# gmlwns2000/sea-attention

Hardware: AMD Instinct MI355X
Metric: tokens/sec + achieved HBM GB/s, OPT-1.3B SEA T=4096 k=64, 1/2/4/8 MI355X (higher is better)
Workload: dtype bf16

## Files before the change

sea-attention_amd/_build.py:

```python
import hashlib
import os
import subprocess
from concurrent.futures import ThreadPoolExecutor

PKG_DIR = os.path.dirname(os.path.abspath(__file__))
CSRC = os.path.join(PKG_DIR, "csrc")
OBJ_DIR = os.path.join(PKG_DIR, "build")
LIB_PATH = os.path.join(PKG_DIR, "libsea_hip.so")
SOURCES = ["sea_topk.hip", "sea_attn.hip", "sea_attn_tile.hip", "sea_attn_keyrange.hip", "sea_attn_bwd.hip", "sea_csr_ops.hip",
           "sea_predictor.hip", "sea_performer.hip", "sea_conv.hip", "sea_mlp.hip", "sea_decode.hip"]
HEADERS = [os.path.join(CSRC, "sea_common.hpp"), os.path.join(CSRC, "sea_attn.hpp"), os.path.join(CSRC, "sea_tail.hpp"),
           os.path.join(CSRC, "sea_convfrag.hpp"),
           os.path.join(os.path.dirname(PKG_DIR), "include", "sea_hip.h")]
COMMON_FLAGS = ["--offload-arch=gfx950", "-O3", "-std=c++17", "-fPIC", "-fno-slp-vectorize", "-Wall", "-Wno-unused-function"]
FILE_FLAGS = {"sea_attn_tile.hip": ["-mllvm", "-amdgpu-mfma-vgpr-form=1"],
              "sea_attn_bwd.hip": ["-mllvm", "-amdgpu-mfma-vgpr-form=1"]}


def _hipcc():
    for c in (os.environ.get("HIPCC"), "/opt/rocm/bin/hipcc", "hipcc"):
        if c and (os.path.isabs(c) and os.path.exists(c) or not os.path.isabs(c)):
            return c
    return "hipcc"

# ... 15 lines not shown
    return bool(_sources()) and all(os.path.exists(os.path.join(CSRC, s)) for s in SOURCES) and all(os.path.exists(h) for h in HEADERS)


def is_stale():
    if not os.path.exists(LIB_PATH):
        return True
    if not sources_present():
        return False
    if not os.path.exists(LIB_PATH + ".sha256"):
        return True
    return open(LIB_PATH + ".sha256").read().strip() != source_hash()


def ensure_built(verbose=False):
    if not is_stale():
        return LIB_PATH
    import fcntl
    with open(LIB_PATH + ".lock", "w") as lk:
        fcntl.flock(lk, fcntl.LOCK_EX)
        try:
            if is_stale():
                build_library(verbose=verbose)
        finally:
            fcntl.flock(lk, fcntl.LOCK_UN)
    return LIB_PATH


def build_library(force=False, extra_flags=(), out=None, verbose=False):
    out = out or LIB_PATH
    if not force and out == LIB_PATH and not is_stale():
        return out
    cc = _hipcc()
    custom = bool(extra_flags) or out != LIB_PATH
    os.makedirs(os.path.join(OBJ_DIR, "custom") if custom else OBJ_DIR, exist_ok=True)

    hdr_bytes = b"".join(open(h, "rb").read() for h in HEADERS)

    def compile_one(src):
        flags = [*COMMON_FLAGS, *FILE_FLAGS.get(src, []), *extra_flags]
        key = hashlib.sha256(open(os.path.join(CSRC, src), "rb").read() + hdr_bytes + repr(flags).encode()).hexdigest()[:16]
        stem = os.path.splitext(src)[0]
        obj = os.path.join(os.path.join(OBJ_DIR, "custom") if custom else OBJ_DIR, f"{stem}.{key}.o")
        if os.path.exists(obj) and not force:
            return obj
        tmp_o = obj + f".tmp.{os.getpid()}"
        cmd = [cc, *flags, "-c", os.path.join(CSRC, src), "-o", tmp_o]
        if verbose:
            print(" ".join(cmd), flush=True)
        subprocess.run(cmd, check=True)
        os.replace(tmp_o, obj)
        for f in os.listdir(OBJ_DIR):
            if f.startswith(stem + ".") and f.endswith(".o") and f != os.path.basename(obj) and not custom:
                try:
                    os.remove(os.path.join(OBJ_DIR, f))
                except OSError:
                    pass
        return obj

    with ThreadPoolExecutor(max_workers=min(8, os.cpu_count() or 1)) as ex:
        objs = list(ex.map(compile_one, _sources()))
    tmp = out + f".tmp.{os.getpid()}"
    cmd = [cc, "--offload-arch=gfx950", "-shared", "-fPIC", *objs, "-o", tmp]
    if verbose:
        print(" ".join(cmd), flush=True)
    subprocess.run(cmd, check=True)
    os.replace(tmp, out)
    if out == LIB_PATH and not extra_flags:
        with open(LIB_PATH + ".sha256", "w") as f:
            f.write(source_hash())
    return out


if __name__ == "__main__":
    print(build_library(force=True, verbose=True))
```

sea-attention_amd/csrc/sea_performer.hip:

```cpp
#include "sea_common.hpp"
#include <cstdlib>

#ifdef SEA_STAMP
__device__ unsigned long long sea_dbg_perf[16];
__device__ unsigned long long sea_dbg_wg[2048];
#define PSTAMP(i) do { if (threadIdx.x == 0) { unsigned long long _t = __builtin_amdgcn_s_memtime(); atomicAdd(&sea_dbg_perf[i], _t - _tprev); _tprev = _t; } } while (0)
#define WSTAMP(i) do { if (threadIdx.x == 0 && (STATE_ONLY || blockIdx.y == 0 || blockIdx.y == gridDim.y - 1)) { unsigned long long _t = __builtin_amdgcn_s_memtime(); _tacc[i] += _t - _tprev; _tprev = _t; } } while (0)
#define WSTAMP_FLUSH() do { if (!STATE_ONLY && threadIdx.x == 0 && (blockIdx.y == 0 || blockIdx.y == gridDim.y - 1)) for (int _i = 0; _i < 4; ++_i) atomicAdd(&sea_dbg_perf[_i + (blockIdx.y ? 0 : 4)], _tacc[_i]); \
    if (STATE_ONLY && threadIdx.x == 0) for (int _i = 0; _i < 4; ++_i) atomicAdd(&sea_dbg_perf[10 + _i], _tacc[_i]); \
    if (threadIdx.x == 0) atomicAdd(&sea_dbg_perf[STATE_ONLY ? 8 : 9], __builtin_amdgcn_s_memtime() - _tstart); \
    if (!STATE_ONLY && threadIdx.x == 0) { const int _w = blockIdx.y * gridDim.x + blockIdx.x; if (_w < 1024) { sea_dbg_wg[2 * _w] = _rstart; sea_dbg_wg[2 * _w + 1] = __builtin_amdgcn_s_memrealtime(); } } } while (0)
#else
#define PSTAMP(i) do {} while (0)
#define WSTAMP(i) do {} while (0)
#define WSTAMP_FLUSH() do {} while (0)
#endif

namespace sea {

using f4 = __attribute__((ext_vector_type(4))) float;
#define SEA_MFMA(a, b, c) __builtin_amdgcn_mfma_f32_16x16x4f32((a), (b), (c), 0, 0, 0)

struct PerfParams {
  const void *q, *k, *v;
// ... 300 lines not shown
    __syncthreads();
    PSTAMP(4);
  }
  if constexpr (STATE_ONLY) {
    float* cw = p.carry + ((int64_t)nh * (p.nseg - 1) + seg) * CARRY;
#pragma unroll
    for (int a = 0; a < JB; ++a)
#pragma unroll
      for (int b = 0; b < NBT; ++b)
#pragma unroll
        for (int r = 0; r < 4; ++r) cw[((a * NBT + b) * 4 + r) * NTH + tid] = S[a][b][r];
    if (tid < NBP) cw[JB * NBT * 4 * NTH + tid] = sKsum[tid];
  } else if (p.state_out && seg == p.nseg - 1) {
    float* cw = p.state_out + (int64_t)nh * CARRY;
#pragma unroll
    for (int a = 0; a < JB; ++a)
#pragma unroll
      for (int b = 0; b < NBT; ++b)
#pragma unroll
        for (int r = 0; r < 4; ++r) cw[((a * NBT + b) * 4 + r) * NTH + tid] = S[a][b][r];
    if (tid < NBP) cw[JB * NBT * 4 * NTH + tid] = sKsum[tid];
  }
}


template <typename T> __device__ inline void split16(float x, unsigned short& hi, unsigned short& lo) {
  hi = S16<T>::bits(x);
  lo = S16<T>::bits(x - S16<T>::val(hi));
}
__device__ inline uint2 pack4(const unsigned short (&v)[4]) {
  return make_uint2((uint32_t)v[0] | ((uint32_t)v[1] << 16), (uint32_t)v[2] | ((uint32_t)v[3] << 16));
}
__device__ inline uint4 cat8(uint2 a, uint2 b) { return make_uint4(a.x, a.y, b.x, b.y); }
__device__ inline uint2 lds_tr(const unsigned short* p) {
  const ps4 v = __builtin_amdgcn_ds_read_tr16_b64_v4i16((ps4 __attribute__((address_space(3)))*)(p));
  return __builtin_bit_cast(uint2, v);
}

template <typename T, int NBT, bool STATE_ONLY, bool SEQ = false, bool PAGED = false>
__global__ __launch_bounds__(512) void performer_bf16_kernel(PerfParams p) {
  constexpr int D = 64, C = 64, NW = 8, NTH = 512, E = 2 * D;
  constexpr int NBP = NBT * 16;
  constexpr int KF = (NBT + 1) / 2;
  constexpr int FP = KF * 32;
  constexpr int RB = C / 16, EB = E / 16;
  static_assert(EB == NW, "one 16-column block of [pos | v] per wave");
  constexpr int LDQ2 = FP + 16;
  constexpr int LDK2 = (FP == 64) ? 96 : FP + 8;
  constexpr int LDA = C + 16;
  constexpr int DSL = RB + NTH / C;
  extern __shared__ __attribute__((aligned(16))) char smem_b[];
  unsigned short* sW = reinterpret_cast<unsigned short*>(smem_b);
  unsigned short* sQ = sW + (D / 8) * NBP * 8;
  unsigned short* sK = sQ + (D / 8) * C * 8;
  unsigned short* sV = sK + (D / 8) * C * 8;
  unsigned short* sQh = sV + C * E;
  unsigned short* sQl = sQh + C * LDQ2;
  unsigned short* sKh = sQl + C * LDQ2;
  unsigned short* sKl = sKh + C * LDK2;
  constexpr int NSET = (FP == 64) ? 2 : 1;
  unsigned short* sAh = sKl + C * LDK2 + (NSET - 1) * (2 * C * LDQ2 + 2 * C * LDK2);
  unsigned short* sAl = sAh + C * LDA;
  float* sKsum = reinterpret_cast<float*>(sAl + C * LDA);
  float* sDenP = sKsum + FP;
  float* sKsP = sDenP + C * DSL;

// ... 99 lines not shown
  auto tril_frag = [&](int ib, int ks) {
    unsigned short o[8];
#pragma unroll
    for (int j = 0; j < 8; ++j) o[j] = (ks * 32 + lg * 8 + j <= ib * 16 + li) ? S16<T>::ONE : (unsigned short)0;
    const unsigned short (&o0)[4] = *reinterpret_cast<const unsigned short (*)[4]>(&o[0]);
    const unsigned short (&o1)[4] = *reinterpret_cast<const unsigned short (*)[4]>(&o[4]);
    return cat8(pack4(o0), pack4(o1));
  };

  uint4 tril[RB][C / 32];
#pragma unroll
  for (int ib = 0; ib < RB; ++ib)
#pragma unroll
    for (int ks = 0; ks < C / 32; ++ks) tril[ib][ks] = tril_frag(ib, ks);

  auto write_state = [&]() {
    float* cw = p.state_out + (int64_t)nh * CARRY;
#pragma unroll
    for (int b = 0; b < NBT; ++b)
#pragma unroll
      for (int r = 0; r < 4; ++r) cw[(b * 4 + r) * NTH + tid] = S[b][r];
    if (tid < FP) cw[NBT * 4 * NTH + tid] = sKsum[tid];
    cw[NBT * 4 * NTH + FP + tid] = li == 0 ? csum[0] : li == 1 ? csum[1] : li == 2 ? csum[2] : li == 3 ? csum[3] : 0.f;
  };

  auto rows_of = [&](int t0) { return min(C, t_end - t0); };
  auto upd_of = [&](int t0) { return !(p.aligned && rows_of(t0) < C); };
  auto stage_qk = [&]() {
    *reinterpret_cast<bu4*>(sQ + (sc * C + (sr ^ (2 * sc))) * 8) = pq;
    *reinterpret_cast<bu4*>(sK + (sc * C + (sr ^ (2 * sc))) * 8) = pk;
  };
  auto stage_v = [&](int t0) {
    const int rows = rows_of(t0);
    if (!STATE_ONLY) __builtin_amdgcn_raw_buffer_store_b128(pv, ro, (sr < rows && t0 + sr >= lead) ? ((t0 + sr) * (3 * D) + 2 * D + sc * 8) * 2 : (int)OOB, 0, 0);
    *reinterpret_cast<bu4*>(sV + sr * E + vchunk(sr, sc) * 8) = pp;
    *reinterpret_cast<bu4*>(sV + sr * E + vchunk(sr, D / 8 + sc) * 8) = pv;
  };
  auto phase_b = [&](int rows, unsigned short* sQh, unsigned short* sQl, unsigned short* sKh, unsigned short* sKl) {
    if (!STATE_ONLY || wv >= RB) {
      const int which = wv / RB, rb = wv - which * RB;
      const unsigned short* src = which ? sK : sQ;
      f4 acc[NBT];
#pragma unroll
      for (int fb = 0; fb < NBT; ++fb) acc[fb] = f4{0.f, 0.f, 0.f, 0.f};
#pragma unroll
      for (int ks = 0; ks < D / 32; ++ks) {
        const uint4 bx = *reinterpret_cast<const uint4*>(src + ((4 * ks + lg) * C + ((rb * 16 + li) ^ (2 * (4 * ks + lg)))) * 8);
#pragma unroll
        for (int fb = 0; fb < NBT; ++fb) {
          const uint4 aw = *reinterpret_cast<const uint4*>(sW + ((4 * ks + lg) * NBP + fb * 16 + li) * 8);
          acc[fb] = S16<T>::mfma(aw, bx, acc[fb]);
        }
      }
      unsigned short* dh = which ? sKh : sQh;
      unsigned short* dl = which ? sKl : sQl;
      const int row = rb * 16 + li;
#pragma unroll
      for (int fb = 0; fb < NBT; ++fb) {
        unsigned short hh[4], ll[4];
#pragma unroll
        for (int r = 0; r < 4; ++r) {
          const int f = fb * 16 + lg * 4 + r;
          float val = fmaxf(cnorm * acc[fb][r], 0.f) + 1e-3f;
          if (f >= p.nb || row >= rows) val = 0.f;
          split16<T>(val, hh[r], ll[r]);
        }
        const int pos = (fb >> 1) * 32 + lg * 8 + (fb & 1) * 4;
// ... 50 lines not shown
        s = fmaf(S16<T>::val((unsigned short)(qh.x & 0xffff)) + S16<T>::val((unsigned short)(ql.x & 0xffff)), ks.x + 1e-6f, s);
        s = fmaf(S16<T>::val((unsigned short)(qh.x >> 16)) + S16<T>::val((unsigned short)(ql.x >> 16)), ks.y + 1e-6f, s);
        s = fmaf(S16<T>::val((unsigned short)(qh.y & 0xffff)) + S16<T>::val((unsigned short)(ql.y & 0xffff)), ks.z + 1e-6f, s);
        s = fmaf(S16<T>::val((unsigned short)(qh.y >> 16)) + S16<T>::val((unsigned short)(ql.y >> 16)), ks.w + 1e-6f, s);
      }
      sDenP[row * DSL + RB + part] = s;
      constexpr int FG = FP / 4, RRN = 64 / FG, RPL = (C / NW) / RRN;
      const int fc = lane % FG, rr = lane / FG;
      float k4[4] = {0.f, 0.f, 0.f, 0.f};
      if (rr < RRN) {
#pragma unroll
        for (int j = 0; j < RPL; ++j) {
          const int r2 = wv * (C / NW) + rr * RPL + j;
          const uint2 kh = *reinterpret_cast<const uint2*>(sKh + r2 * LDK2 + fc * 4);
          const uint2 kl = *reinterpret_cast<const uint2*>(sKl + r2 * LDK2 + fc * 4);
          k4[0] += S16<T>::val((unsigned short)(kh.x & 0xffff)) + S16<T>::val((unsigned short)(kl.x & 0xffff));
          k4[1] += S16<T>::val((unsigned short)(kh.x >> 16)) + S16<T>::val((unsigned short)(kl.x >> 16));
          k4[2] += S16<T>::val((unsigned short)(kh.y & 0xffff)) + S16<T>::val((unsigned short)(kl.y & 0xffff));
          k4[3] += S16<T>::val((unsigned short)(kh.y >> 16)) + S16<T>::val((unsigned short)(kl.y >> 16));
        }
      }
#pragma unroll
      for (int j = 0; j < 4; ++j) {
        if constexpr (FG == 16) {
          k4[j] = xor16_sum(xor32_sum(k4[j]));
        } else {
#pragma unroll
          for (int o = FG * (RRN / 2); o >= FG; o >>= 1) k4[j] += __shfl_down(k4[j], o);
        }
      }
      if (lane < FG) *reinterpret_cast<float4*>(sKsP + wv * FP + fc * 4) = make_float4(k4[0], k4[1], k4[2], k4[3]);
    }
  };
  auto phase_de = [&](int t0, int rows, bool upd, const unsigned short* sQh, const unsigned short* sQl, const unsigned short* sKh,
                      const unsigned short* sKl) {
    if (tid < FP) {
      float s = sKsum[tid];
#pragma unroll
      for (int i = 0; i < NW; ++i) s += sKsP[i * FP + tid];
      if (upd) sKsum[tid] = s;
    }
    float dn[RB], ri1 = 0.f;
    if constexpr (!STATE_ONLY) {
      const int myrow = (lg % RB) * 16 + li;
      float s = 0.f;
#pragma unroll
      for (int i = 0; i < DSL; ++i) s += sDenP[myrow * DSL + i];
      const float d1 = 1.0f / s;
      ri1 = 1.0f / (float)(row_base + t0 + myrow + 1);
#pragma unroll
      for (int ib = 0; ib < RB; ++ib) dn[ib] = __shfl(d1, ib * 16 + li);
    }
    {
      const int jb = wv, e0 = jb * 16;
      uint4 vf[C / 32];
      {
        const int q = li >> 2, pp_ = li & 3;
#pragma unroll
        for (int ks = 0; ks < C / 32; ++ks) {
          const int r0 = ks * 32 + lg * 8;
          const uint2 a = lds_tr(sV + (r0 + q) * E + vchunk(r0 + q, 2 * jb + (pp_ >> 1)) * 8 + 4 * (pp_ & 1));
          const uint2 b = lds_tr(sV + (r0 + 4 + q) * E + vchunk(r0 + 4 + q, 2 * jb + (pp_ >> 1)) * 8 + 4 * (pp_ & 1));
          vf[ks] = cat8(a, b);
        }
      }
      if constexpr (STATE_ONLY) {
        if (want_avg && jb >= EB / 2) {
          f4 cum = f4{0.f, 0.f, 0.f, 0.f};
#pragma unroll
          for (int ks = 0; ks <= (RB - 1) / 2; ++ks) cum = S16<T>::mfma(vf[ks], tril[RB - 1][ks], cum);
#pragma unroll
          for (int r = 0; r < 4; ++r) csum[r] += __shfl(cum[r], (lane & 48) | 15);
        }
      } else {
      f4 o[RB];
#pragma unroll
      for (int ib = 0; ib < RB; ++ib) o[ib] = f4{0.f, 0.f, 0.f, 0.f};
#pragma unroll
      for (int ib = 0; ib < RB; ++ib) {
#pragma unroll
        for (int ks = 0; ks <= ib / 2; ++ks) {
          const uint4 ah = *reinterpret_cast<const uint4*>(sAh + (ib * 16 + li) * LDA + ks * 32 + lg * 8);
          const uint4 al = *reinterpret_cast<const uint4*>(sAl + (ib * 16 + li) * LDA + ks * 32 + lg * 8);
          o[ib] = S16<T>::mfma(vf[ks], ah, o[ib]);
          o[ib] = S16<T>::mfma(vf[ks], al, o[ib]);
        }
      }
#pragma unroll
      for (int kk = 0; kk < KF; ++kk) {
        unsigned short h0[4], h1[4], l0[4], l1[4];
#pragma unroll
        for (int r = 0; r < 4; ++r) {
          split16<T>(S[2 * kk][r], h0[r], l0[r]);
          if (2 * kk + 1 < NBT) split16<T>(S[(2 * kk + 1 < NBT) ? 2 * kk + 1 : 0][r], h1[r], l1[r]);
          else h1[r] = l1[r] = 0;
        }
        const uint4 bh = cat8(pack4(h0), pack4(h1)), bl = cat8(pack4(l0), pack4(l1));
#pragma unroll
        for (int ib = 0; ib < RB; ++ib) {
          const uint4 ah = *reinterpret_cast<const uint4*>(sQh + (ib * 16 + li) * LDQ2 + kk * 32 + lg * 8);
          const uint4 al = *reinterpret_cast<const uint4*>(sQl + (ib * 16 + li) * LDQ2 + kk * 32 + lg * 8);
          o[ib] = S16<T>::mfma(bh, ah, o[ib]);
          o[ib] = S16<T>::mfma(bl, ah, o[ib]);
          o[ib] = S16<T>::mfma(bh, al, o[ib]);
        }
      }
      const int col = e0 + 4 * lg;
#pragma unroll
      for (int ib = 0; ib < RB; ++ib) {
        const int row = ib * 16 + li;
        unsigned short ob[4];
#pragma unroll
        for (int r = 0; r < 4; ++r) ob[r] = S16<T>::bits(o[ib][r] * dn[ib]);
        const uint2 w2 = pack4(ob);
        typedef __attribute__((ext_vector_type(2))) unsigned int bu2;
        __builtin_amdgcn_raw_buffer_store_b64(bu2{w2.x, w2.y}, ro, (row < rows && t0 + row >= lead) ? ((t0 + row) * (3 * D) + col) * 2 : (int)OOB, 0, 0);
      }
      if (want_avg && jb >= EB / 2) {
        f4 cum[RB];
#pragma unroll
        for (int ib = 0; ib < RB; ++ib) {
          cum[ib] = f4{0.f, 0.f, 0.f, 0.f};
#pragma unroll
          for (int ks = 0; ks <= ib / 2; ++ks) cum[ib] = S16<T>::mfma(vf[ks], tril[ib][ks], cum[ib]);
        }
        const int gcol = col - D;
#pragma unroll
        for (int ib = 0; ib < RB; ++ib) {
          const int row = ib * 16 + li;
          const float ri = __shfl(ri1, ib * 16 + li);
          unsigned short gb4[4];
#pragma unroll
          for (int r = 0; r < 4; ++r) gb4[r] = S16<T>::bits((cum[ib][r] + csum[r]) * ri);
          const uint2 w2 = pack4(gb4);
          typedef __attribute__((ext_vector_type(2))) unsigned int bu2;
          __builtin_amdgcn_raw_buffer_store_b64(bu2{w2.x, w2.y}, rg, (row < rows && t0 + row >= lead) ? ((t0 + row) * D + gcol) * 2 : (int)OOB, 0, 0);
        }
        if (upd) {
#pragma unroll
          for (int r = 0; r < 4; ++r) csum[r] += __shfl(cum[RB - 1][r], (lane & 48) | 15);
        }
      }
      }
      if (upd) {
        const int q = li >> 2, pp_ = li & 3;
#pragma unroll
        for (int rb = 0; rb < NBT; ++rb) {
#pragma unroll
          for (int ks = 0; ks < C / 32; ++ks) {
            const int r0 = ks * 32 + lg * 8;
            const int co = (rb >> 1) * 32 + 8 * pp_ + (rb & 1) * 4;
            const uint4 kh = cat8(lds_tr(sKh + (r0 + q) * LDK2 + co), lds_tr(sKh + (r0 + 4 + q) * LDK2 + co));
            const uint4 kl = cat8(lds_tr(sKl + (r0 + q) * LDK2 + co), lds_tr(sKl + (r0 + 4 + q) * LDK2 + co));
            S[rb] = S16<T>::mfma(kh, vf[ks], S[rb]);
            S[rb] = S16<T>::mfma(kl, vf[ks], S[rb]);
          }
        }
      }
    }
  };
  constexpr int PHI = 2 * C * LDQ2 + 2 * C * LDK2;
  auto run_b = [&](int t0, int buf) { phase_b(rows_of(t0), sQh + buf * PHI, sQl + buf * PHI, sKh + buf * PHI, sKl + buf * PHI); };
  auto run_c = [&](int buf) { phase_c(sQh + buf * PHI, sQl + buf * PHI, sKh + buf * PHI, sKl + buf * PHI); };
  auto run_de = [&](int t0, int buf) {
    phase_de(t0, rows_of(t0), upd_of(t0), sQh + buf * PHI, sQl + buf * PHI, sKh + buf * PHI, sKl + buf * PHI);
  };
  if (t_begin < t_end) {
    stage_qk();
    stage_v(t_begin);
    issue_qk(t_begin + C);
    issue_v(t_begin + C);
    __syncthreads();
    run_b(t_begin, 0);
    __syncthreads();
    run_c(0);
    stage_qk();
    issue_qk(t_begin + 2 * C);
    __syncthreads();
    int buf = 0;
    for (int t0 = t_begin; t0 < t_end; t0 += C, buf ^= (NSET - 1)) {
      const bool has_next = t0 + C < t_end;
      run_de(t0, buf);
      if constexpr (NSET == 1) __syncthreads();
      if (has_next) run_b(t0 + C, buf ^ (NSET - 1));
      __syncthreads();
      PSTAMP(0);
      if (has_next) {
        run_c(buf ^ (NSET - 1));
        stage_v(t0 + C);
        issue_v(t0 + 2 * C);
        stage_qk();
        issue_qk(t0 + 3 * C);
      }
      __syncthreads();
      PSTAMP(1);
    }
  }
  if constexpr (STATE_ONLY) {
    float* cw = p.carry + ((int64_t)nh * (p.nseg - 1) + seg) * CARRY;
#pragma unroll
    for (int b = 0; b < NBT; ++b)
#pragma unroll
      for (int r = 0; r < 4; ++r) cw[(b * 4 + r) * NTH + tid] = S[b][r];
    if (tid < FP) cw[NBT * 4 * NTH + tid] = sKsum[tid];
    cw[NBT * 4 * NTH + FP + tid] = li == 0 ? csum[0] : li == 1 ? csum[1] : li == 2 ? csum[2] : li == 3 ? csum[3] : 0.f;
  } else {
    const bool unchanged = p.aligned && p.state_in == p.state_out && t_end - t_begin <= C && !upd_of(t_begin);
    if (p.state_out && seg == p.nseg - 1 && !unchanged) write_state();
#ifdef SEA_STAMP
    if (threadIdx.x == 0) { const int _w = blockIdx.y * gridDim.x + blockIdx.x; if (_w < 1024) { sea_dbg_wg[2 * _w] = _rstart64; sea_dbg_wg[2 * _w + 1] = __builtin_amdgcn_s_memrealtime(); } }
#endif
  }
}

template <typename T, int D, int C, int NBT, bool STATE_ONLY, bool SEQ = false, bool PAGED = false>
__global__ __launch_bounds__(512) void performer_bf16w_kernel(PerfParams p) {
  constexpr int NW = 8, NTH = 512, E = 2 * D, CPR = D / 8;
// ... 86 lines not shown
        for (int r = 0; r < 4; ++r) csum[jq][r] = cr[JB * NBT * 4 * NTH + FP + jq * NTH + cslot + r];
      }
      if (tid < FP) ks0 = cr[JB * NBT * 4 * NTH + tid];
    }
    if (!STATE_ONLY) {
      for (int s2 = 0; s2 < seg; ++s2) {
        const float* cr = p.carry + ((int64_t)nh * (p.nseg - 1) + s2) * CARRY;
#pragma unroll
        for (int jq = 0; jq < JB; ++jq) {
#pragma unroll
          for (int b = 0; b < NBT; ++b)
#pragma unroll
            for (int r = 0; r < 4; ++r) S[jq][b][r] += cr[((jq * NBT + b) * 4 + r) * NTH + tid];
#pragma unroll
          for (int r = 0; r < 4; ++r) csum[jq][r] += cr[JB * NBT * 4 * NTH + FP + jq * NTH + cslot + r];
        }
        if (tid < FP) ks0 += cr[JB * NBT * 4 * NTH + tid];
      }
    }
    if (tid < FP) sKsum[tid] = ks0;
  }

  if constexpr (SEQ) { if (tb < 0) return; }
  const bool stager = tid >= NTH - STG;
  const int stid = stager ? tid - (NTH - STG) : 0;
  const int sr = stid / CPR, sc = stid - sr * CPR;
  constexpr unsigned OOB = 0x7FFFFF00u;
  auto mk = [&](const T* base, int64_t row_stride) {
    return __builtin_amdgcn_make_buffer_rsrc(const_cast<T*>(base), 0, (int)(((int64_t)(TL - 1) * row_stride + D) * 2), 0x00020000);
  };
  const __amdgpu_buffer_rsrc_t rq = mk(qb, p.qs[2]), rk = mk(kb, p.ks[2]), rv = mk(vb, p.vs[2]), rp = mk(pb, p.pos_stride);
  const __amdgpu_buffer_rsrc_t ro = __builtin_amdgcn_make_buffer_rsrc(ob, 0, (int)((int64_t)TL * 3 * D * 2), 0x00020000);
  typedef __attribute__((ext_vector_type(4))) unsigned int bu4;
  typedef __attribute__((ext_vector_type(2))) unsigned int bu2;
  const bool want_avg = p.avg != nullptr;
  T* gb = reinterpret_cast<T*>(p.avg) + (want_avg ? (int64_t)nh * p.T * D - (int64_t)lead * D : 0);
  const __amdgpu_buffer_rsrc_t rg = __builtin_amdgcn_make_buffer_rsrc(gb, 0, want_avg ? (int)((int64_t)TL * D * 2) : 0, 0x00020000);
  struct Pre { bu4 q, k, v, p; };
  Pre pa, pn;
  auto issue_qk = [&](int t0n, Pre& r) {
    const int t = t0n + sr;
    const bool ok = t < t_end && stager;
    r.q = __builtin_amdgcn_raw_buffer_load_b128(rq, (ok && !STATE_ONLY && t >= lead) ? (int)((t * p.qs[2] + sc * 8) * 2) : (int)OOB, 0, 0);
    r.k = __builtin_amdgcn_raw_buffer_load_b128(rk, ok ? (int)((t * p.ks[2] + sc * 8) * 2) : (int)OOB, 0, 0);
  };
  auto issue_v = [&](int t0n, Pre& r) {
    const int t = t0n + sr;
    const bool ok = t < t_end && stager;
    r.v = __builtin_amdgcn_raw_buffer_load_b128(rv, ok ? (int)((t * p.vs[2] + sc * 8) * 2) : (int)OOB, 0, 0);
    r.p = __builtin_amdgcn_raw_buffer_load_b128(rp, ok ? (int)((t * p.pos_stride + sc * 8) * 2) : (int)OOB, 0, 0);
  };
  issue_qk(t_begin, pa);
  issue_v(t_begin, pa);
  auto vchunk = [](int row, int ch) { return ch ^ ((((row & 3) | (((row >> 3) & 1) << 2))) << 1); };

  auto tril_frag = [&](int ib, int ks) {
    unsigned short o[8];
#pragma unroll
    for (int j = 0; j < 8; ++j) o[j] = (ks * 32 + lg * 8 + j <= ib * 16 + li) ? S16<T>::ONE : (unsigned short)0;
    const unsigned short (&o0)[4] = *reinterpret_cast<const unsigned short (*)[4]>(&o[0]);
    const unsigned short (&o1)[4] = *reinterpret_cast<const unsigned short (*)[4]>(&o[4]);
    return cat8(pack4(o0), pack4(o1));
  };

  uint4 tril[RB][C / 32];
#pragma unroll
  for (int ib = 0; ib < RB; ++ib)
// ... 206 lines not shown
      } else {
      f4 o[RB];
#pragma unroll
      for (int ib = 0; ib < RB; ++ib) o[ib] = f4{0.f, 0.f, 0.f, 0.f};
#pragma unroll
      for (int ib = 0; ib < RB; ++ib) {
#pragma unroll
        for (int ks = 0; ks <= ib / 2; ++ks) {
          const uint4 ah = *reinterpret_cast<const uint4*>(sAh + (ib * 16 + li) * LDA + ks * 32 + lg * 8);
          const uint4 al = *reinterpret_cast<const uint4*>(sAl + (ib * 16 + li) * LDA + ks * 32 + lg * 8);
          o[ib] = S16<T>::mfma(vf[ks], ah, o[ib]);
          o[ib] = S16<T>::mfma(vf[ks], al, o[ib]);
        }
      }
#pragma unroll
      for (int kk = 0; kk < KF; ++kk) {
        unsigned short h0[4], h1[4], l0[4], l1[4];
#pragma unroll
        for (int r = 0; r < 4; ++r) {
          split16<T>(S[jq][2 * kk][r], h0[r], l0[r]);
          if (2 * kk + 1 < NBT) split16<T>(S[jq][(2 * kk + 1 < NBT) ? 2 * kk + 1 : 0][r], h1[r], l1[r]);
          else h1[r] = l1[r] = 0;
        }
        const uint4 bh = cat8(pack4(h0), pack4(h1)), bl = cat8(pack4(l0), pack4(l1));
#pragma unroll
        for (int ib = 0; ib < RB; ++ib) {
          const uint4 ah = *reinterpret_cast<const uint4*>(sQh + (ib * 16 + li) * LDQ2 + kk * 32 + lg * 8);
          const uint4 al = *reinterpret_cast<const uint4*>(sQl + (ib * 16 + li) * LDQ2 + kk * 32 + lg * 8);
          o[ib] = S16<T>::mfma(bh, ah, o[ib]);
          o[ib] = S16<T>::mfma(bl, ah, o[ib]);
          o[ib] = S16<T>::mfma(bh, al, o[ib]);
        }
      }
      const int col = e0 + 4 * lg;
#pragma unroll
      for (int ib = 0; ib < RB; ++ib) {
        const int row = ib * 16 + li;
        unsigned short o4[4];
#pragma unroll
        for (int r = 0; r < 4; ++r) o4[r] = S16<T>::bits(o[ib][r] * dn[ib]);
        const uint2 w2 = pack4(o4);
        __builtin_amdgcn_raw_buffer_store_b64(bu2{w2.x, w2.y}, ro, (row < rows && t0 + row >= lead) ? ((t0 + row) * (3 * D) + col) * 2 : (int)OOB, 0, 0);
      }
      if (want_avg && jb >= EB / 2) {
        f4 cum[RB];
#pragma unroll
        for (int ib = 0; ib < RB; ++ib) {
          cum[ib] = f4{0.f, 0.f, 0.f, 0.f};
#pragma unroll
          for (int ks = 0; ks <= ib / 2; ++ks) cum[ib] = S16<T>::mfma(vf[ks], tril[ib][ks], cum[ib]);
        }
        const int gcol = col - D;
#pragma unroll
        for (int ib = 0; ib < RB; ++ib) {
          const int row = ib * 16 + li;
          const float ri = __shfl(ri1, ib * 16 + li);
          unsigned short g4[4];
#pragma unroll
          for (int r = 0; r < 4; ++r) g4[r] = S16<T>::bits((cum[ib][r] + csum[jq][r]) * ri);
          const uint2 w2 = pack4(g4);
          __builtin_amdgcn_raw_buffer_store_b64(bu2{w2.x, w2.y}, rg, (row < rows && t0 + row >= lead) ? ((t0 + row) * D + gcol) * 2 : (int)OOB, 0, 0);
        }
        if (upd) {
#pragma unroll
          for (int r = 0; r < 4; ++r) csum[jq][r] += __shfl(cum[RB - 1][r], (lane & 48) | 15);
        }
      }
      }
      if (upd) {
        const int q = li >> 2, pp_ = li & 3;
#pragma unroll
        for (int rb = 0; rb < NBT; ++rb) {
#pragma unroll
          for (int ks = 0; ks < C / 32; ++ks) {
            const int r0 = ks * 32 + lg * 8;
            const int co = (rb >> 1) * 32 + 8 * pp_ + (rb & 1) * 4;
            const uint4 kh = cat8(lds_tr(sKh + (r0 + q) * LDK2 + co), lds_tr(sKh + (r0 + 4 + q) * LDK2 + co));
            const uint4 kl = cat8(lds_tr(sKl + (r0 + q) * LDK2 + co), lds_tr(sKl + (r0 + 4 + q) * LDK2 + co));
            S[jq][rb] = S16<T>::mfma(kh, vf[ks], S[jq][rb]);
            S[jq][rb] = S16<T>::mfma(kl, vf[ks], S[jq][rb]);
          }
        }
      }
    }
  };
  if constexpr (STATE_ONLY) {
    auto stage_k_to = [&](unsigned short* dst, const bu4& r) {
      if (stager) *reinterpret_cast<bu4*>(dst + (sc * C + (sr ^ sc)) * 8) = r;
    };
    auto stage_v_to = [&](unsigned short* dst, const bu4& rp_, const bu4& rv_) {
      if (stager) {
        *reinterpret_cast<bu4*>(dst + sr * EL + vchunk(sr, sc) * 8) = rp_;
        *reinterpret_cast<bu4*>(dst + sr * EL + vchunk(sr, CPR + sc) * 8) = rv_;
      }
    };
// ... 494 lines not shown
```

sea-attention_amd/csrc/sea_topk.hip:

```cpp
#include "sea_common.hpp"
#include "sea_tail.hpp"
#include "sea_convfrag.hpp"


#ifdef SEA_STAMP
__device__ unsigned long long sea_dbg[16];
#define STAMP(i) do { if (threadIdx.x == 0) { unsigned long long _t = __builtin_amdgcn_s_memtime(); \
  atomicAdd(&sea_dbg[i], _t - _tprev); _tprev = _t; } } while (0)
#else
#define STAMP(i) do {} while (0)
#endif

namespace sea {

constexpr int TK_THREADS = 256;
constexpr int TK_WAVES = TK_THREADS / WAVE;
constexpr int TK_MAX_BINS = 2048;

__device__ inline uint32_t f2key(float f) {
  f = f + 0.0f;
  uint32_t u = __float_as_uint(f);
  return u ^ ((u >> 31) ? 0xFFFFFFFFu : 0x80000000u);
}

// ... 125 lines not shown
    for (int e = 0; e < 4; ++e) cnt += (valid && k4[e] == tau) ? 1 : 0;
    int total = 0, rank = 0;
    if (n_eq != r) rank = seen + block_excl_scan(cnt, s_wave, &total);
    for (int e = 0; e < 4; ++e) {
      if (!valid) continue;
      if (k4[e] > tau) sel |= 1ull << (4 * j + e);
      if (k4[e] == tau) {
        if (n_eq == r || rank < r) sel |= 1ull << (4 * j + e);
        ++rank;
      }
    }
    seen += total;
  }
  return sel;
}

__device__ inline long long block_excl_scan64(long long v, long long* s_wave , long long* total) {
  const int lane = threadIdx.x & 63, w = threadIdx.x >> 6;
  long long incl = wave_incl_scan(v);
  if (lane == 63) s_wave[w] = incl;
  __syncthreads();
  long long base = 0, tot = 0;
#pragma unroll
  for (int i = 0; i < TK_WAVES; ++i) {
    const long long x = s_wave[i];
    if (i < w) base += x;
    tot += x;
  }
  __syncthreads();
  *total = tot;
  return base + incl - v;
}

template <typename T, int EPT, bool FROM_MASK, bool FULL, int HMAX = 1024, bool EXT_CAND = false, bool K16 = false, bool HCW = K16>
__device__ __forceinline__ void select_body(const TopkParams& p, uint32_t (&key)[K16 ? EPT / 2 : EPT], unsigned long long sel, int n,
                                            int t, int row, const T* base, uint32_t* cand = nullptr) {
  constexpr int R = EPT / 4;
  static_assert(!K16 || (sizeof(T) == 2 && !FROM_MASK), "packed keys: 16-bit maps");
  auto key_at = [&](int i) -> uint32_t {
    if constexpr (K16) return (i & 1) ? (key[i >> 1] >> 16) : (key[i >> 1] & 0xffffu);
    else return key[i];
  };
  auto digit_at = [&](int i, int shift, int d) -> int {
    if constexpr (K16) return (int)__builtin_amdgcn_ubfe(~key[i >> 1], shift + 16 * (i & 1), d);
    else return (int)__builtin_amdgcn_ubfe(~key[i], shift, d);
  };
  __shared__ int s_hist[TK_MAX_BINS + 1];
  __shared__ int s_head[HMAX];
  __shared__ int s_wave[TK_WAVES];
  __shared__ uint32_t s_red[2 * TK_WAVES];
  __shared__ int s_bcast[4];
  uint32_t* s_ckey;
  uint32_t* s_cidx;
  if constexpr (EXT_CAND) {
    s_ckey = cand; s_cidx = cand + TK_CAND_CAP;
  } else {
    __shared__ uint32_t s_cand[2 * TK_CAND_CAP];
    s_ckey = s_cand; s_cidx = s_cand + TK_CAND_CAP;
  }
  __shared__ uint32_t s_selbits[512];
  __shared__ int s_ncand;

  const int tid = threadIdx.x;
  const int lane = tid & 63, wv = tid >> 6;
#ifdef SEA_STAMP
  unsigned long long _tprev = __builtin_amdgcn_s_memtime();
// ... 155 lines not shown
#pragma unroll
          for (int e = 0; e < 4; ++e) {
            tie[e] = in_bin(4 * j + e) && (key_at(4 * j + e) & lowmask) == tau_low;
            cnt += tie[e] ? 1 : 0;
          }
          int total = 0, rank = 0;
          if (n_eq != kth) rank = seen + block_excl_scan(cnt, s_wave, &total);
#pragma unroll
          for (int e = 0; e < 4; ++e) {
            if (tie[e]) {
              if (n_eq == kth || rank < kth) sel |= 1ull << (4 * j + e);
              ++rank;
            }
          }
          seen += total;
        }
        __syncthreads();
      } else {
        sel = select_multipass<T>(base, p.sh, p.T_m, p.nchunks, p.M, K, umin, umax, R, s_hist, s_wave, s_bcast);
        for (int i = tid; i < p.H; i += TK_THREADS) s_head[i] = 0;
        __syncthreads();
      }
    }
  } else {
    __syncthreads();
  }

  STAMP(3);
  const int w_t = row_width(t, p.T_dst, p.t_src_dev ? p.t_src_dev[n * p.t_src_stride] : p.T_src, p.is_causal);
  const float scale = interp_scale(w_t, p.T_m);
  const bool tm_pow2 = (p.T_m & (p.T_m - 1)) == 0;
  const int tm_sh = __ffs(p.T_m) - 1;
#pragma unroll
  for (int j = 0; j < R; ++j) {
    const int c = j * TK_THREADS + tid;
    const bool valid = FULL || c < p.nchunks;
    const uint32_t nib = (uint32_t)(sel >> (4 * j)) & 0xFu;
    uint32_t word = nib << (4 * (lane & 7));
    word |= dpp_u32<0xB1>(word);
    word |= dpp_u32<0x4E>(word);
    word |= dpp_u32<0x141>(word);
    if ((lane & 7) == 0 && (c >> 3) < p.W) p.bits[(int64_t)row * p.W + (c >> 3)] = word;
    if (p.mask_out != nullptr && valid) {
      const int f0 = c * 4;
      const int h = f0 / p.T_m, b0 = f0 - h * p.T_m;
      float4 m;
      m.x = (nib & 1u) ? 1.f : 0.f; m.y = (nib & 2u) ? 1.f : 0.f;
      m.z = (nib & 4u) ? 1.f : 0.f; m.w = (nib & 8u) ? 1.f : 0.f;
      *reinterpret_cast<float4*>(p.mask_out + (((int64_t)n * p.H + h) * p.T_dst + t) * p.T_m + b0) = m;
    }
  }
  if constexpr (K16 && HCW) {
    int wpx[4];
    {
      float bprev = interp_bound(4 * lane, scale);
#pragma unroll
      for (int e = 0; e < 4; ++e) {
        const float bnext = interp_bound(4 * lane + e + 1, scale);
        const int w = (int)(bnext - bprev);
        wpx[e] = w < p.max_k ? w : p.max_k;
        bprev = bnext;
      }
    }
#pragma unroll
    for (int j0 = 0; j0 < R; j0 += 8) {
      float red[8];
#pragma unroll
      for (int b = 0; b < 8; ++b) {
        int sum = 0;
        if (j0 + b < R) {
          const uint32_t nib = (uint32_t)(sel >> (4 * (j0 + b))) & 0xFu;
#pragma unroll
          for (int e = 0; e < 4; ++e) sum += (nib >> e) & 1u ? wpx[e] : 0;
        }
        red[b] = (float)sum;
// ... 1134 lines not shown
```

Before: 15.41 million.

## Widen performer output stores via permlane16 pairing and transpose top-k bitmask writes

The performer kernels now pack pairs of 16-row query blocks with permlane16_swap, so each lane issues 128-bit buffer stores instead of 64-bit ones for the O and averaged-V outputs. An optional late-store mode defers these writes until after the next stage's work. In the top-k selection kernel, the bitmask words are built with an 8-lane nibble transpose, so every lane writes one word rather than one lane in eight after an OR-reduction. The change also adds compile-time experiment switches that drop stores, plus caching of custom builds. Cross-lane permutes and extra code paths are added in exchange for fewer and wider memory transactions.

```diff
diff --git a/sea-attention_amd/_build.py b/sea-attention_amd/_build.py
--- a/sea-attention_amd/_build.py
+++ b/sea-attention_amd/_build.py
@@ -71,6 +71,10 @@
         return out
     cc = _hipcc()
     custom = bool(extra_flags) or out != LIB_PATH
+    stamp = hashlib.sha256((source_hash() + repr(tuple(extra_flags))).encode()).hexdigest()
+    if custom and not force and os.path.exists(out) and os.path.exists(out + ".sha256") \
+            and open(out + ".sha256").read().strip() == stamp:
+        return out
     os.makedirs(os.path.join(OBJ_DIR, "custom") if custom else OBJ_DIR, exist_ok=True)
 
     hdr_bytes = b"".join(open(h, "rb").read() for h in HEADERS)
@@ -107,6 +111,9 @@
     if out == LIB_PATH and not extra_flags:
         with open(LIB_PATH + ".sha256", "w") as f:
             f.write(source_hash())
+    elif custom:
+        with open(out + ".sha256", "w") as f:
+            f.write(stamp)
     return out
 
 
diff --git a/sea-attention_amd/csrc/sea_performer.hip b/sea-attention_amd/csrc/sea_performer.hip
--- a/sea-attention_amd/csrc/sea_performer.hip
+++ b/sea-attention_amd/csrc/sea_performer.hip
@@ -356,6 +356,53 @@
   return make_uint2((uint32_t)v[0] | ((uint32_t)v[1] << 16), (uint32_t)v[2] | ((uint32_t)v[3] << 16));
 }
 __device__ inline uint4 cat8(uint2 a, uint2 b) { return make_uint4(a.x, a.y, b.x, b.y); }
+#ifndef SEA_PERF_NARROW_STORES
+#define SEA_PERF_WIDE_STORES 1
+#else
+#define SEA_PERF_WIDE_STORES 0
+#endif
+typedef __attribute__((ext_vector_type(2))) unsigned int perf_u2;
+typedef __attribute__((ext_vector_type(4))) unsigned int perf_u4;
+__device__ inline perf_u4 pair16(uint2 a, uint2 b) {
+  const auto x = __builtin_amdgcn_permlane16_swap(a.x, b.x, false, false);
+  const auto y = __builtin_amdgcn_permlane16_swap(a.y, b.y, false, false);
+  return perf_u4{x[0], y[0], x[1], y[1]};
+}
+template <int RB, bool DROP>
+__device__ inline void store_blocks(const uint2 (&w)[RB], __amdgpu_buffer_rsrc_t rs, int t0, int rows, int lead, int ld, int col,
+                                    int li, int lg) {
+  constexpr unsigned OOB = 0x7FFFFF00u;
+  if constexpr (DROP) {
+    uint32_t x = 0;
+#pragma unroll
+    for (int ib = 0; ib < RB; ++ib) x ^= w[ib].x ^ (w[ib].y * 3u);
+    if (x == 0x12345678u && rows < 0) __builtin_amdgcn_raw_buffer_store_b32(x, rs, 0, 0, 0);
+    return;
+  }
+  static_assert(RB % 2 == 0, "query blocks leave in pairs");
+#pragma unroll
+  for (int ib = 0; ib < RB; ib += 2) {
+    const int row = (ib + (lg & 1)) * 16 + li;
+    __builtin_amdgcn_raw_buffer_store_b128(pair16(w[ib], w[ib + 1]), rs,
+        (row < rows && t0 + row >= lead) ? ((t0 + row) * ld + col + 4 * (lg & ~1)) * 2 : (int)OOB, 0, 0);
+  }
+}
+#ifdef SEA_PERF_EXP_NOSTORE_O
+[[maybe_unused]] constexpr bool PERF_DROP_O = true;
+#else
+[[maybe_unused]] constexpr bool PERF_DROP_O = false;
+#endif
+#ifdef SEA_PERF_EXP_NOSTORE_AVG
+[[maybe_unused]] constexpr bool PERF_DROP_AVG = true;
+#else
+[[maybe_unused]] constexpr bool PERF_DROP_AVG = false;
+#endif
+#ifdef SEA_PERF_EXP_NOSTORE_V
+[[maybe_unused]] constexpr bool PERF_DROP_V = true;
+#else
+[[maybe_unused]] constexpr bool PERF_DROP_V = false;
+#endif
+
 __device__ inline uint2 lds_tr(const unsigned short* p) {
   const ps4 v = __builtin_amdgcn_ds_read_tr16_b64_v4i16((ps4 __attribute__((address_space(3)))*)(p));
   return __builtin_bit_cast(uint2, v);
@@ -521,7 +568,7 @@
   };
   auto stage_v = [&](int t0) {
     const int rows = rows_of(t0);
-    if (!STATE_ONLY) __builtin_amdgcn_raw_buffer_store_b128(pv, ro, (sr < rows && t0 + sr >= lead) ? ((t0 + sr) * (3 * D) + 2 * D + sc * 8) * 2 : (int)OOB, 0, 0);
+    if (!STATE_ONLY && !PERF_DROP_V) __builtin_amdgcn_raw_buffer_store_b128(pv, ro, (sr < rows && t0 + sr >= lead) ? ((t0 + sr) * (3 * D) + 2 * D + sc * 8) * 2 : (int)OOB, 0, 0);
     *reinterpret_cast<bu4*>(sV + sr * E + vchunk(sr, sc) * 8) = pp;
     *reinterpret_cast<bu4*>(sV + sr * E + vchunk(sr, D / 8 + sc) * 8) = pv;
   };
@@ -638,6 +685,16 @@
       if (lane < FG) *reinterpret_cast<float4*>(sKsP + wv * FP + fc * 4) = make_float4(k4[0], k4[1], k4[2], k4[3]);
     }
   };
+#if defined(SEA_PERF_LATE_STORES) && SEA_PERF_WIDE_STORES
+  constexpr bool LATE = !STATE_ONLY;
+#elif SEA_PERF_WIDE_STORES
+  constexpr bool LATE = false;
+#endif
+#if SEA_PERF_WIDE_STORES
+  uint2 wo[RB], wg[RB];
+  auto store_o = [&](int t0, int rows) { store_blocks<RB, PERF_DROP_O>(wo, ro, t0, rows, lead, 3 * D, wv * 16, li, lg); };
+  auto store_g = [&](int t0, int rows) { store_blocks<RB, PERF_DROP_AVG>(wg, rg, t0, rows, lead, D, wv * 16 - D, li, lg); };
+#endif
   auto phase_de = [&](int t0, int rows, bool upd, const unsigned short* sQh, const unsigned short* sQl, const unsigned short* sKh,
                       const unsigned short* sKl) {
     if (tid < FP) {
@@ -658,7 +715,7 @@
       for (int ib = 0; ib < RB; ++ib) dn[ib] = __shfl(d1, ib * 16 + li);
     }
     {
-      const int jb = wv, e0 = jb * 16;
+      const int jb = wv;
       uint4 vf[C / 32];
       {
         const int q = li >> 2, pp_ = li & 3;
@@ -711,7 +768,17 @@
           o[ib] = S16<T>::mfma(bh, al, o[ib]);
         }
       }
-      const int col = e0 + 4 * lg;
+#if SEA_PERF_WIDE_STORES
+#pragma unroll
+      for (int ib = 0; ib < RB; ++ib) {
+        unsigned short ob[4];
+#pragma unroll
+        for (int r = 0; r < 4; ++r) ob[r] = S16<T>::bits(o[ib][r] * dn[ib]);
+        wo[ib] = pack4(ob);
+      }
+      if constexpr (!LATE) store_o(t0, rows);
+#else
+      const int col = wv * 16 + 4 * lg;
 #pragma unroll
       for (int ib = 0; ib < RB; ++ib) {
         const int row = ib * 16 + li;
@@ -719,9 +786,9 @@
 #pragma unroll
         for (int r = 0; r < 4; ++r) ob[r] = S16<T>::bits(o[ib][r] * dn[ib]);
         const uint2 w2 = pack4(ob);
-        typedef __attribute__((ext_vector_type(2))) unsigned int bu2;
-        __builtin_amdgcn_raw_buffer_store_b64(bu2{w2.x, w2.y}, ro, (row < rows && t0 + row >= lead) ? ((t0 + row) * (3 * D) + col) * 2 : (int)OOB, 0, 0);
-      }
+        __builtin_amdgcn_raw_buffer_store_b64(perf_u2{w2.x, w2.y}, ro, (row < rows && t0 + row >= lead) ? ((t0 + row) * (3 * D) + col) * 2 : (int)OOB, 0, 0);
+      }
+#endif
       if (want_avg && jb >= EB / 2) {
         f4 cum[RB];
 #pragma unroll
@@ -730,6 +797,17 @@
 #pragma unroll
           for (int ks = 0; ks <= ib / 2; ++ks) cum[ib] = S16<T>::mfma(vf[ks], tril[ib][ks], cum[ib]);
         }
+#if SEA_PERF_WIDE_STORES
+#pragma unroll
+        for (int ib = 0; ib < RB; ++ib) {
+          const float ri = __shfl(ri1, ib * 16 + li);
+          unsigned short gb4[4];
+#pragma unroll
+          for (int r = 0; r < 4; ++r) gb4[r] = S16<T>::bits((cum[ib][r] + csum[r]) * ri);
+          wg[ib] = pack4(gb4);
+        }
+        if constexpr (!LATE) store_g(t0, rows);
+#else
         const int gcol = col - D;
 #pragma unroll
         for (int ib = 0; ib < RB; ++ib) {
@@ -739,9 +817,9 @@
 #pragma unroll
           for (int r = 0; r < 4; ++r) gb4[r] = S16<T>::bits((cum[ib][r] + csum[r]) * ri);
           const uint2 w2 = pack4(gb4);
-          typedef __attribute__((ext_vector_type(2))) unsigned int bu2;
-          __builtin_amdgcn_raw_buffer_store_b64(bu2{w2.x, w2.y}, rg, (row < rows && t0 + row >= lead) ? ((t0 + row) * D + gcol) * 2 : (int)OOB, 0, 0);
-        }
+          __builtin_amdgcn_raw_buffer_store_b64(perf_u2{w2.x, w2.y}, rg, (row < rows && t0 + row >= lead) ? ((t0 + row) * D + gcol) * 2 : (int)OOB, 0, 0);
+        }
+#endif
         if (upd) {
 #pragma unroll
           for (int r = 0; r < 4; ++r) csum[r] += __shfl(cum[RB - 1][r], (lane & 48) | 15);
@@ -789,6 +867,12 @@
       run_de(t0, buf);
       if constexpr (NSET == 1) __syncthreads();
       if (has_next) run_b(t0 + C, buf ^ (NSET - 1));
+#if SEA_PERF_WIDE_STORES
+      if constexpr (LATE) {
+        store_o(t0, rows_of(t0));
+        if (want_avg && wv >= EB / 2) store_g(t0, rows_of(t0));
+      }
+#endif
       __syncthreads();
       PSTAMP(0);
       if (has_next) {
@@ -941,7 +1025,6 @@
   const __amdgpu_buffer_rsrc_t rq = mk(qb, p.qs[2]), rk = mk(kb, p.ks[2]), rv = mk(vb, p.vs[2]), rp = mk(pb, p.pos_stride);
   const __amdgpu_buffer_rsrc_t ro = __builtin_amdgcn_make_buffer_rsrc(ob, 0, (int)((int64_t)TL * 3 * D * 2), 0x00020000);
   typedef __attribute__((ext_vector_type(4))) unsigned int bu4;
-  typedef __attribute__((ext_vector_type(2))) unsigned int bu2;
   const bool want_avg = p.avg != nullptr;
   T* gb = reinterpret_cast<T*>(p.avg) + (want_avg ? (int64_t)nh * p.T * D - (int64_t)lead * D : 0);
   const __amdgpu_buffer_rsrc_t rg = __builtin_amdgcn_make_buffer_rsrc(gb, 0, want_avg ? (int)((int64_t)TL * D * 2) : 0, 0x00020000);
@@ -1214,6 +1297,17 @@
           o[ib] = S16<T>::mfma(bh, al, o[ib]);
         }
       }
+#if SEA_PERF_WIDE_STORES
+      uint2 wo[RB];
+#pragma unroll
+      for (int ib = 0; ib < RB; ++ib) {
+        unsigned short o4[4];
+#pragma unroll
+        for (int r = 0; r < 4; ++r) o4[r] = S16<T>::bits(o[ib][r] * dn[ib]);
+        wo[ib] = pack4(o4);
+      }
+      store_blocks<RB, PERF_DROP_O>(wo, ro, t0, rows, lead, 3 * D, e0, li, lg);
+#else
       const int col = e0 + 4 * lg;
 #pragma unroll
       for (int ib = 0; ib < RB; ++ib) {
@@ -1222,8 +1316,9 @@
 #pragma unroll
         for (int r = 0; r < 4; ++r) o4[r] = S16<T>::bits(o[ib][r] * dn[ib]);
         const uint2 w2 = pack4(o4);
-        __builtin_amdgcn_raw_buffer_store_b64(bu2{w2.x, w2.y}, ro, (row < rows && t0 + row >= lead) ? ((t0 + row) * (3 * D) + col) * 2 : (int)OOB, 0, 0);
-      }
+        __builtin_amdgcn_raw_buffer_store_b64(perf_u2{w2.x, w2.y}, ro, (row < rows && t0 + row >= lead) ? ((t0 + row) * (3 * D) + col) * 2 : (int)OOB, 0, 0);
+      }
+#endif
       if (want_avg && jb >= EB / 2) {
         f4 cum[RB];
 #pragma unroll
@@ -1232,6 +1327,18 @@
 #pragma unroll
           for (int ks = 0; ks <= ib / 2; ++ks) cum[ib] = S16<T>::mfma(vf[ks], tril[ib][ks], cum[ib]);
         }
+#if SEA_PERF_WIDE_STORES
+        uint2 wg[RB];
+#pragma unroll
+        for (int ib = 0; ib < RB; ++ib) {
+          const float ri = __shfl(ri1, ib * 16 + li);
+          unsigned short g4[4];
+#pragma unroll
+          for (int r = 0; r < 4; ++r) g4[r] = S16<T>::bits((cum[ib][r] + csum[jq][r]) * ri);
+          wg[ib] = pack4(g4);
+        }
+        store_blocks<RB, PERF_DROP_AVG>(wg, rg, t0, rows, lead, D, e0 - D, li, lg);
+#else
         const int gcol = col - D;
 #pragma unroll
         for (int ib = 0; ib < RB; ++ib) {
@@ -1241,8 +1348,9 @@
 #pragma unroll
           for (int r = 0; r < 4; ++r) g4[r] = S16<T>::bits((cum[ib][r] + csum[jq][r]) * ri);
           const uint2 w2 = pack4(g4);
-          __builtin_amdgcn_raw_buffer_store_b64(bu2{w2.x, w2.y}, rg, (row < rows && t0 + row >= lead) ? ((t0 + row) * D + gcol) * 2 : (int)OOB, 0, 0);
-        }
+          __builtin_amdgcn_raw_buffer_store_b64(perf_u2{w2.x, w2.y}, rg, (row < rows && t0 + row >= lead) ? ((t0 + row) * D + gcol) * 2 : (int)OOB, 0, 0);
+        }
+#endif
         if (upd) {
 #pragma unroll
           for (int r = 0; r < 4; ++r) csum[jq][r] += __shfl(cum[RB - 1][r], (lane & 48) | 15);
diff --git a/sea-attention_amd/csrc/sea_topk.hip b/sea-attention_amd/csrc/sea_topk.hip
--- a/sea-attention_amd/csrc/sea_topk.hip
+++ b/sea-attention_amd/csrc/sea_topk.hip
@@ -181,6 +181,16 @@
   return base + incl - v;
 }
 
+__device__ __forceinline__ uint32_t nib_transpose8(uint32_t v, int lane) {
+  uint32_t q = dpp_u32<0xB1>(v);
+  v = (lane & 1) ? (v & 0xF0F0F0F0u) | ((q >> 4) & 0x0F0F0F0Fu) : (v & 0x0F0F0F0Fu) | ((q << 4) & 0xF0F0F0F0u);
+  q = dpp_u32<0x4E>(v);
+  v = (lane & 2) ? (v & 0xFF00FF00u) | ((q >> 8) & 0x00FF00FFu) : (v & 0x00FF00FFu) | ((q << 8) & 0xFF00FF00u);
+  q = dpp_u32<0x1B>(dpp_u32<0x141>(v));
+  v = (lane & 4) ? (v & 0xFFFF0000u) | (q >> 16) : (v & 0x0000FFFFu) | (q << 16);
+  return v;
+}
+
 template <typename T, int EPT, bool FROM_MASK, bool FULL, int HMAX = 1024, bool EXT_CAND = false, bool K16 = false, bool HCW = K16>
 __device__ __forceinline__ void select_body(const TopkParams& p, uint32_t (&key)[K16 ? EPT / 2 : EPT], unsigned long long sel, int n,
                                             int t, int row, const T* base, uint32_t* cand = nullptr) {
@@ -402,15 +412,21 @@
   const bool tm_pow2 = (p.T_m & (p.T_m - 1)) == 0;
   const int tm_sh = __ffs(p.T_m) - 1;
 #pragma unroll
+  for (int j0 = 0; j0 < R; j0 += 8) {
+    const uint32_t mine = nib_transpose8((uint32_t)(sel >> (4 * j0)), lane);
+    const int jm = j0 + (lane & 7);
+    const int wi = (jm * TK_THREADS + tid) >> 3;
+#ifndef SEA_SEL_EXP_NOSTORE
+    if (jm < R && wi < p.W) p.bits[(int64_t)row * p.W + wi] = mine;
+#else
+    if (mine == 0x12345678u && wi < -p.W) p.bits[(int64_t)row * p.W] = mine;
+#endif
+  }
+#pragma unroll
   for (int j = 0; j < R; ++j) {
     const int c = j * TK_THREADS + tid;
     const bool valid = FULL || c < p.nchunks;
     const uint32_t nib = (uint32_t)(sel >> (4 * j)) & 0xFu;
-    uint32_t word = nib << (4 * (lane & 7));
-    word |= dpp_u32<0xB1>(word);
-    word |= dpp_u32<0x4E>(word);
-    word |= dpp_u32<0x141>(word);
-    if ((lane & 7) == 0 && (c >> 3) < p.W) p.bits[(int64_t)row * p.W + (c >> 3)] = word;
     if (p.mask_out != nullptr && valid) {
       const int f0 = c * 4;
       const int h = f0 / p.T_m, b0 = f0 - h * p.T_m;
```

After: 15.45 million (median of 3 runs). About the same (+0.3%).
